# SJTU-ViSYS/TextSLAM

Measured on AMD Instinct MI355X. Metric: local_ba_residuals_per_s, higher is better.
Workload: dtype f64; 1 GPU; C4 local BA: 20 KF x 5000 pts x 100 text planes (541 (KF,plane) pairs x 64 features), passes 2,1,0 x <=10 LM its; parallelism=1 GPU, resid_evals_per_call=8113350

## Files before the change

### textslam_amd/csrc/tsba.hip

```cpp
#include <hip/hip_runtime.h>
#include <cstdio>
#include <cstdlib>
#include <cstring>
#include <cmath>
#include <string>
#include <vector>
#include <chrono>
#include <thread>
#include <mutex>
#include <map>
#include <condition_variable>
#include <atomic>
#include <functional>
#include <dlfcn.h>
#include <rccl/rccl.h>
#include "../../include/tsba.h"
#include "../../include/tsba_debug.h"
#include "tsba_device.h"
#include "tsraster.h"
#include "tsquadstat.h"
#include "tsba_plan.h"

#include "tsba_types.h"
#include "tsba_kernels_lin.h"
// ... 486 lines not shown
                set_err(c, "hipHostMalloc (plane cache staging)"); return TSBA_ERR_DEVICE; }
            IC.stage_cap = need; }
        for (size_t m = 0; m < miss.size(); m++) { const int k = miss[m];
            for (int l = 0; l < p->n_levels; l++) if (mask >> l & 1) memcpy(IC.stage + m*off + lo[l], p->img[l][k], (size_t)p->img_w[l]*p->img_h[l]);
            hipMemcpyAsync(IC.dev + (size_t)ic_slot[(size_t)k]*off, IC.stage + m*off, off, hipMemcpyHostToDevice, c->stream); }
    }
    c->use_img_cache = true;
    return 0;
}
static int stage_levels(Ctx *c, const tsba_problem *p, const tsba_options *o, const PlanStart &S, LevelMax *mx, UploadTimes &T) {
    if (S.first_plan) {
        flush_run(c);
        const auto tp0 = UpClock::now(); S.first_plan();
        T.plan += ms_between(tp0, UpClock::now()); }
    const std::vector<int> used = levels_used(o, p->n_levels);
    for (size_t i = 0; i < used.size(); i++) {
        const int l = used[i];
        if (S.defer && i > 0) { mx->take(level_capacity(p, l)); continue; }
        const int rc = stage_level(c, p, l, &T.plan, &T.img); if (rc) return rc;
        mx->take(level_size(c->lev[l]));
    }
    c->stage_p = S.defer ? p : nullptr;
    return 0;
}
static int alloc_pose_buffers(Ctx *c, const tsba_problem *p, const LevelMax &mx) {
    Work &W = c->W;
    c->pose_only = p->n_kf == 1 && every_landmark_frozen(p) && !c->dbg.no_pose_kernel;
    W.pst = nullptr; W.ppart = nullptr;
    if (c->pose_only) { AL(W.pst, 2); AL(W.ppart, 3*28*mx.pose_grid); }
    return 0;
}
static int alloc_lin_buffers(Ctx *c, const tsba_problem *p, const LevelMax &mx) {
    Work &W = c->W;
    for (int b = 0; b < 2; b++) {
        LinBuf &B = W.lb[b];
        AL(B.pairM, 27*mx.pair); AL(B.pairCost, mx.pair); AL(B.pairR, 9*mx.pair); AL(B.pairOut, 90*mx.pair);
        AL(B.tgM, 27*mx.tg); AL(B.tgCost, mx.tg);
        AL(B.w_pt, PT_REC*mx.pslot); AL(B.vdb_pt, PT_VDB*(size_t)p->n_pt);
        AL(B.w_tx, TX_REC*mx.tslot); AL(B.V_tx, 6*(size_t)p->n_text); AL(B.b_tx, 3*(size_t)p->n_text); AL(B.dgs_tx, 3*(size_t)p->n_text);
        AL(B.Hd, W.N); AL(B.bp, W.N); AL(B.bp_loc, W.N); AL(B.dgs_p, W.N);
        AL(B.lmpart, 3*((size_t)p->n_pt/64 + (size_t)p->n_text/2 + mx.pair + 8));
    }
    AL(W.sig_pt, p->n_pt); AL(W.sig_tx, 3*(size_t)p->n_text); AL(W.sig_p, W.N);
    AL(W.cb, 2*(size_t)W.N + 8); AL(W.cbm, 1);
    return 0;
}
static SolverLayout upload_layout(const Ctx *c) {
    int ring = 0, ring_k0 = 0; for (int l = 0; l < c->n_levels; l++) if (c->lev_built[l] && c->hplan[l].ring) { ring = 1; ring_k0 = c->hplan[l].ring_k0; }
    return choose_solver_layout(c->n_kf, max_band_rows(c), ring, ring_k0, is_multi(c), c->dbg);
}
static int alloc_reduced_system(Ctx *c, const tsba_problem *p, const SolverLayout &L) {
    Work &W = c->W; const int bw = L.bw_rows;
    c->lay = L;
    W.dp_poll = L.use_lds && !is_multi(c) && !c->pose_only && (c->dbg.solve_variant == 0 || c->dbg.solve_variant == 5 || c->dbg.solve_variant == 6);
    if (W.dp_poll) {
        const int ldsb = solve_back_lds_bytes((int)(solve_lds_doubles(W.N)*sizeof(double)), W.N);
        ATTR(k_solve_back<true>, ldsb);
        if (!grid_resident(c, (const void *)k_solve_back<true>, SOLVE_THREADS, (size_t)ldsb, 1 + (c->nb_back_max + 2)/3)) W.dp_poll = 0;
    }
    c->S_up = L.S_up; c->S_count = L.S_count; AL(c->S_alloc, c->S_count);
    if (!L.band) { W.S = c->S_alloc; W.ldS = W.N; W.band = 0; }
    else { W.S = c->S_alloc + (L.LDB - L.S_up); W.ldS = (int)L.LDB - 1; W.band = 1; }
    W.ring = 0; W.ring_g = 0; W.ring_b = 0; W.ring_k0 = -1;
    c->Lcol = nullptr; c->band_stream = L.band_stream; c->sep_cr = L.sep_cr != 0; c->band_parts = L.P;
    if (L.band_stream) AL(c->Lcol, ((size_t)p->n_kf + bw/6 + 1)*bw*6);
    if (L.partitioned) {
        const int P = L.P, nsep = L.nsep;
        c->nsep_ld = nsep;
        AL(c->Lb, ((size_t)p->n_kf + bw/6 + 1)*bw*6); AL(c->Tbuf, (size_t)P*((size_t)4*bw*bw + 2*bw));
        AL(c->Bpart, (size_t)P*BANDP_NS*((size_t)bw*bw + bw));
        if (L.sep_cr) { AL(c->Ssep, cr_pool_blocks(L.nsepb)*(size_t)bw*bw); AL(c->CRcontrib, (size_t)L.nsepb*cre_contrib_doubles(bw)); AL(c->CRfac, (size_t)L.nsepb*cre_rec_doubles(bw)); AL(c->CRgate, (size_t)(L.nsepb + 2)*TSBA_CRE_KMAX); c->cre_epoch = 0; }
        else AL(c->Ssep, (size_t)nsep*nsep + nsep);
        AL(c->Lcol_sep, (size_t)(nsep/6 + 1)*L.bws*6);
        Work &Ws = c->Wsep; memset(&Ws, 0, sizeof(Ws));
        Ws.N = nsep; Ws.n_kf = 0; Ws.S = c->Ssep; Ws.ldS = nsep; Ws.band = 1; Ws.st = nullptr;
        AL(Ws.Sy, nsep); AL(Ws.g, nsep); AL(Ws.dp, nsep); AL(Ws.LDbuf, 32*(size_t)(nsep/6 + 1)); AL(Ws.nfree, 1); AL(Ws.fidx, 1);
        W.ring = L.ring; W.ring_g = L.ring_G; W.ring_b = bw/6; W.ring_k0 = L.ring_k0;
    }
    if (L.err) { set_err(c, "ring-shaped map: the partitioned band solver is not available for this plan"); return L.err; }
    AL(W.Sy, W.N + BAND_BW_MAX);
    return 0;
}
static int alloc_pcg(Ctx *c, const tsba_problem *p, const SolverLayout &L) {
    Work &W = c->W;
    c->far_B = 0; c->n_far = 0; c->pcg_parts = 0;
    for (int l = 0; l < p->n_levels; l++) if (c->lev_built[l] && c->lev[l].far_B > 0) { c->far_B = c->lev[l].far_B; c->n_far = std::max(c->n_far, c->lev[l].n_far); }
    if (c->far_B > 0) {
        if (!W.band || !c->band_stream) { set_err(c, "map with long-range coupling: the band solvers are not available for this plan"); return TSBA_ERR_STATE; }
        c->pcg_parts = (p->n_kf + 31)/32;
        AL(W.Sfar, 36*(size_t)std::max(c->n_far, 1));
        AL(W.pc_x, W.N); AL(W.pc_r, W.N); AL(W.pc_p[0], W.N); AL(W.pc_p[1], W.N); AL(W.pc_q, W.N); AL(W.pc_g0, W.N);
        AL(W.pc_part, 5*(size_t)c->pcg_parts + 16 + 144); AL(W.pcs, 2); AL(W.pc_stat, 8);
    }
    c->S_xchg = nullptr; c->xchg_wp = L.xchg_wp;
    if (L.xchg_wp) AL(c->S_xchg, ((size_t)W.N + L.bw_rows)*L.xchg_wp);
    return 0;
}
static int alloc_step_buffers(Ctx *c, const tsba_problem *p, const LevelMax &mx) {
    Work &W = c->W;
    AL(W.g, W.N); AL(W.dp, W.N + 2); AL(W.dl_pt, p->n_pt); AL(W.dl_tx, 3*(size_t)p->n_text);
    AL(W.partial, 2*(size_t)c->nb_back_max);
    AL(W.posepart, 2*((size_t)p->n_kf/21 + 2));
    AL(W.cntpart, 2*(mx.cnt/4 + mx.cnt/256 + 4));
    AL(W.st, 2); c->st_base = W.st; AL(W.dec, 1);
    W.st_next = (W.dp_poll && p->n_kf <= SCHUR_KEEP_KF) ? W.st + 1 : nullptr;
    AL(c->cov_log, 6*TSBA_MAX_LEVELS);
    return 0;
// ... 242 lines not shown
        c->lin_base += grid;
        return;
    }
    if (D.n_pair + D.n_tg > 0) launch_k_linearize(c, D, spec);
    const MidDec md0{0, 0, 0, tsba_options{}};
    if (mid_threads(c) == MID_TW) LAUNCHK((k_mid<MID_TW, 6, MID_PR_MIN>), dim3(nb_pt + nb_tx + nb_pr), dim3(MID_TW), 0, c->stream, W, D, nb_pt, nb_tx, spec, md0);
    else if (mid_threads(c) == 64) {
        const int dec_on = spec && decision_in_mid(c, D) ? 1 : 0;
        LAUNCHK((k_mid<64, 6, MID_PR_MIN>), dim3(nb_pt + nb_tx + nb_pr + dec_on), dim3(64), 0, c->stream, W, D, nb_pt, nb_tx, spec,
                dec_on ? MidDec{1, nb_pr, back_blocks_pt(c->n_pt) + back_blocks_tx(c->n_text) + nb_kf, c->opt} : md0);
    } else LAUNCHK((k_mid<256, 4, MID_PR_MIN>), dim3(nb_pt + nb_tx + nb_pr), dim3(256), 0, c->stream, W, D, nb_pt, nb_tx, spec, md0);
    const int multi = is_multi(c);
    const int npp = pose_parts(c);
    if (multi) {
        if (npp) LAUNCHK(k_pose_sums_raw, dim3(npp), dim3(256), 0, c->stream, W, D, spec);
        LAUNCHK(k_sums_multi, dim3(1), dim3(256), 0, c->stream, W, D, spec, nb_pt + nb_tx + nb_pr, back_blocks_pt(c->n_pt) + back_blocks_tx(c->n_text) + nb_kf, back_blocks_pt(c->n_pt) + back_blocks_tx(c->n_text), npp);
        allreduce(c, W.cb, 2*(size_t)W.N + 8, ncclDouble, ncclSum);
        allreduce(c, W.cbm, 1, ncclDouble, ncclMax);
        if (npp) LAUNCHK(k_pose_scale_multi, dim3(npp), dim3(256), 0, c->stream, W, spec);
    } else if (npp) LAUNCHK(k_pose_sums, dim3(npp), dim3(256), 0, c->stream, W, D, spec);
    if (!spec && !skip_postlin) LAUNCHK(k_postlin, dim3(1), dim3(256), 0, c->stream, W, D, c->opt.gradient_tolerance, nb_pt + nb_tx + nb_pr, multi, npp);
}
static int solve_lds_bytes(Ctx *c, int *use_lds) {
    *use_lds = lds_solver_fits(c->W.N);
    return *use_lds ? (int)(solve_lds_doubles(c->W.N)*sizeof(double)) : 0;
}
static int chol_subst_lds_bytes() { return (CH_NB*(CH_NB + 1) + 2*CH_NB + 8*CH_NB)*(int)sizeof(double); }
static void launch_schur(Ctx *c, const LevelDev &D, int multi, SchurDec dec = SchurDec{0, 0, 0, tsba_options{}}) {
    if (c->n_kf > 126 && !c->dbg.no_schur_quad) {
        const int nq = D.n_sb > 0 ? (((D.n_sb + 3)/4 + 7)/8)*8 : 0, ng = ((c->n_kf + 7)/8)*8;
        if (D.n_tg > 0) LAUNCHK(k_schur_quad<true>, dim3(nq + ng), dim3(64), 0, c->stream, c->W, D, multi, nq, ng);
        else LAUNCHK(k_schur_quad<false>, dim3(nq + ng), dim3(64), 0, c->stream, c->W, D, multi, nq, ng);
    } else if (c->n_kf > 126) LAUNCHK(k_schur_t<1>, dim3(D.n_sb + c->n_kf), dim3(64), 0, c->stream, c->W, D, multi, 0, SchurDec{0, 0, 0, tsba_options{}});
    else LAUNCHK(k_schur_t<4>, dim3(D.n_sb + c->n_kf + (dec.on == 3 ? 1 : 0)), dim3(256), 0, c->stream, c->W, D, multi, 0, dec);
    if (D.far_B > 0 && D.n_far > 0) {
        LevelDev E = D;
        E.n_sb = D.n_far; E.sb_a = D.far_a; E.sb_b = D.far_b; E.sb_pab = D.fb_pab; E.sb_pba = D.fb_pba; E.sb_far = D.fb_id;
        E.sb_pt_off = D.fb_pt_off; E.sb_pt_s1 = D.fb_pt_s1; E.sb_pt_s2 = D.fb_pt_s2; E.sb_pt_lm = D.fb_pt_lm;
        E.sb_tx_off = D.fb_tx_off; E.sb_tx_s1 = D.fb_tx_s1; E.sb_tx_s2 = D.fb_tx_s2; E.sb_tx_lm = D.fb_tx_lm;
        if (c->n_kf > 126 && !c->dbg.no_schur_quad) { const int nq = (((E.n_sb + 3)/4 + 7)/8)*8;
            if (D.n_tg > 0) LAUNCHK(k_schur_quad<true>, dim3(nq), dim3(64), 0, c->stream, c->W, E, multi, nq, 0);
            else LAUNCHK(k_schur_quad<false>, dim3(nq), dim3(64), 0, c->stream, c->W, E, multi, nq, 0); }
        else if (c->n_kf > 126) LAUNCHK(k_schur_t<1>, dim3(E.n_sb), dim3(64), 0, c->stream, c->W, E, multi, 0, SchurDec{0, 0, 0, tsba_options{}});
        else LAUNCHK(k_schur_t<4>, dim3(E.n_sb), dim3(256), 0, c->stream, c->W, E, multi, 0, SchurDec{0, 0, 0, tsba_options{}});
    }
}
static int set_solver_attrs(Ctx *c) {
    int use_lds; int lds = solve_lds_bytes(c, &use_lds);
    if (use_lds) { ATTR(k_solve_t<false>, lds);
        ATTR((k_solve_t<false, false>), lds);
        ATTR(k_solve_back<true>, solve_back_lds_bytes(lds, c->W.N));
        ATTR(k_solve_back<false>, solve_back_lds_bytes(lds, c->W.N));
        ATTR((k_solve_back<true, true>), solve_back_lds_bytes(lds, c->W.N));
        ATTR(k_solve_la, (int)std::min<size_t>(solve_la_lds_doubles(c->W.N)*sizeof(double), 160*1024 - 64)); }
    else {
        ATTR(k_band_solve, 156*1024);
        ATTR(k_bandp_factor, 156*1024);
        ATTR(k_cr_pivot, 156*1024);
        ATTR(k_cr_update, 156*1024);
        ATTR(k_cr_back, 156*1024);
        ATTR(k_cre_elim, 156*1024);
        ATTR(k_bandp_sepf, 156*1024);
        ATTR(k_cre_back, 156*1024);
        ATTR(k_ms_cre_back, 159*1024);
        ATTR(k_ms_cre_fwd, 100*1024);
        ATTR(k_ms_cre_root, 100*1024);
        ATTR(k_sv_linv, 156*1024);
#define MX_ATTR(SS) ATTR(k_mx_cre_fwd<SS>, 156*1024); ATTR(k_mx_cre_root<SS>, 156*1024); ATTR(k_mx_cre_back<SS>, 156*1024);
        MX_ATTR(36) MX_ATTR(42) MX_ATTR(48) MX_ATTR(54) MX_ATTR(60) MX_ATTR(66)
#undef MX_ATTR
        ATTR(k_sv_fwd_int<1>, 156*1024); ATTR(k_sv_fwd_int<2>, 156*1024);
        ATTR(k_sv_back_int<1>, 156*1024); ATTR(k_sv_back_int<2>, 156*1024);
        ATTR(k_sv_tree_back<1>, 150*1024); ATTR(k_sv_tree_back<2>, 150*1024);
        ATTR(k_bandp_backsub<1>, 156*1024); ATTR(k_bandp_backsub<2>, 156*1024);
        ATTR(k_band_backsub<1>, 156*1024); ATTR(k_band_backsub<2>, 156*1024); ATTR(k_band_backsub<3>, 156*1024);
        ATTR(k_solve_t<true>, (int)(solve_diag_lds_doubles()*sizeof(double)));
        ATTR(k_chol_panel, (CH_NB + 64)*(CH_NB + 1)*(int)sizeof(double));
        ATTR(k_chol_update, 2*64*(CH_NB + 1)*(int)sizeof(double));
        ATTR(k_chol_backsub, chol_subst_lds_bytes()); ATTR(k_chol_fwd, chol_subst_lds_bytes());
    }
    return 0;
}
#include "tsba_solve_launch.h"

static bool fused_decisions(const Ctx *c, const LevelDev &D) { return c->W.st_next != nullptr && D.far_B <= 0; }
static bool window_fast_ctx(const Ctx *c, bool per_step) { return c->W.st_next != nullptr && c->n_kf <= 64 && !is_multi(c) && !c->pose_only && !per_step; }
static bool window_fast(const Ctx *c, const LevelDev &D, bool per_step) { return window_fast_ctx(c, per_step) && D.far_B <= 0 && D.n_sc + D.n_tg > 0; }
static void launch_decide(Ctx *c, const LevelDev &D) {
    Work &W = c->W;
    int nb_pt, nb_tx, nb_pr; mid_blocks(c, D, nb_pt, nb_tx, nb_pr); const int nb_kf = (c->n_kf + 255)/256;
    const int nb_all = back_blocks_pt(c->n_pt) + back_blocks_tx(c->n_text) + nb_kf;
    LAUNCHK(k_decide, dim3(1), dim3(256), 0, c->stream, W, D, nb_all, nb_pt + nb_tx + nb_pr, c->opt, (int)is_multi(c), pose_parts(c));
}
static void launch_step(Ctx *c, const LevelDev &D, bool decide_prev = false, bool first_fused = false) {
    struct XT { Ctx *c; size_t x0; ~XT() { c->x_trial = c->x_acc - x0; } } xt{c, c->x_acc};
    Work &W = c->W;
    int nb_pt, nb_tx, nb_pr; mid_blocks(c, D, nb_pt, nb_tx, nb_pr); const int nb_kf = (c->n_kf + 255)/256;
    if ((int64_t)D.n_sb < (int64_t)c->n_kf*(c->n_kf + 1)/2 && (!c->band_stream || c->S_stale || is_multi(c))) {
        hipMemsetAsync(c->S_alloc, 0, sizeof(double)*c->S_count, c->stream); c->S_stale = false;
        if (D.far_B > 0) hipMemsetAsync(W.Sfar, 0, sizeof(double)*36*(size_t)std::max(D.n_far, 1), c->stream); }
    const int bb_pt = back_blocks_pt(c->n_pt), bb_tx = back_blocks_tx(c->n_text), nb_all = bb_pt + bb_tx + nb_kf;
    const bool fused_decide = fused_decisions(c, D);
    if (fused_decide && (decide_prev || first_fused)) {
        launch_schur(c, D, 0, SchurDec{decide_prev ? (decision_in_mid(c, D) ? 3 : 1) : 2, nb_all, nb_pt + nb_tx + nb_pr, c->opt});
        std::swap(W.st, W.st_next);
    } else launch_schur(c, D, (int)is_multi(c));
    if (is_multi(c)) {
        if (c->S_xchg) {
            const size_t nx = ((size_t)W.N + (W.ring ? c->xchg_wp - 6 : 0))*c->xchg_wp;
            const int nbp = (int)std::min<size_t>(2048, (nx + 255)/256);
            LAUNCHK(k_band_pack, dim3(nbp), dim3(256), 0, c->stream, W, c->S_xchg, c->xchg_wp, 0);
            allreduce(c, c->S_xchg, nx, ncclDouble, ncclSum);
            LAUNCHK(k_band_pack, dim3(nbp), dim3(256), 0, c->stream, W, c->S_xchg, c->xchg_wp, 1);
        } else allreduce(c, c->S_alloc, c->S_count, ncclDouble, ncclSum);
        if (D.far_B > 0 && D.n_far > 0) allreduce(c, W.Sfar, 36*(size_t)D.n_far, ncclDouble, ncclSum);
        allreduce(c, W.g, W.N, ncclDouble, ncclSum);
        LAUNCHK(k_damp_multi, dim3((c->n_kf + 255)/256), dim3(256), 0, c->stream, W);
    }
    if (W.dp_poll && D.far_B <= 0) {
        int use_lds; const int lds = solve_lds_bytes(c, &use_lds);
        const int ldsb = solve_back_lds_bytes(lds, W.N);
        if (c->dbg.solve_variant == 6) LAUNCHK((k_solve_back<true, true>), dim3(1 + (nb_all + 2)/3), dim3(SOLVE_THREADS), ldsb, c->stream, W, D, bb_pt, bb_tx, nb_all);
        else if (c->dbg.solve_variant == 5) LAUNCHK(k_solve_back<false>, dim3(1 + (nb_all + 2)/3), dim3(SOLVE_THREADS), ldsb, c->stream, W, D, bb_pt, bb_tx, nb_all);
        else LAUNCHK(k_solve_back<true>, dim3(1 + (nb_all + 2)/3), dim3(SOLVE_THREADS), ldsb, c->stream, W, D, bb_pt, bb_tx, nb_all);
    } else {
        launch_solve_full(c, D);
        LAUNCHK(k_back, dim3(nb_all), dim3(256), 0, c->stream, W, D, bb_pt, bb_tx);
    }
    launch_linearize(c, D, 1);
    if (!fused_decide) launch_decide(c, D);
}

struct PassCarry {
    const bool per_step;
    bool log_pending = false;
    int ms_ahead = -1;
    bool clear_part = false;
};
static bool pose_path(const Ctx *c) { return c->pose_only && !is_multi(c); }
static bool converged(const Ctx *c, int it) {
    if (!c->hprog || is_multi(c)) return false;
    const auto tw = std::chrono::steady_clock::now();
    for (int spin = 0;; spin++) {
        const unsigned long long w = *(volatile unsigned long long *)c->hprog;
        if ((unsigned int)(w >> 32) == c->W.pass_seq) { if (w & 1) return true; if ((int)((w & 0xffffffffu) >> 1) + 2 > it) break; }
        else if (it < 2) break;
        PlanPool::cpu_relax();
        if ((spin & 1023) == 1023 && std::chrono::steady_clock::now() - tw > std::chrono::seconds(2)) break;
    }
    return false;
}
static int level_ready(Ctx *c, int l) {
    if (!c->lev_built[l]) {
        if (!c->stage_p) { set_err(c, "level not staged"); return TSBA_ERR_STATE; }
        c->stage_async = true; const int rc = stage_level(c, c->stage_p, l, nullptr, nullptr); c->stage_async = false; if (rc) return rc; }
    if (c->lev_wait[l]) { hipStreamWaitEvent(c->stream, c->ev_stage[l], 0); c->lev_wait[l] = 0; }
    return TSBA_OK;
}
static void record_cov(Ctx *c, int ps) { if (c->cov_text >= 0 && c->cov_text < c->n_text && ps < TSBA_MAX_LEVELS) LAUNCHK(k_record_vtx, dim3(1), dim3(64), 0, c->stream, c->W, c->cov_text, c->cov_log + 6*ps); }
static int pose_pass(Ctx *c, int ps, PassCarry &carry) {
    const tsba_options &o = c->opt; const LevelDev &D = c->lev[o.levels[ps]]; const int G = pose_grid(D);
    const bool one_launch = !carry.per_step && grid_resident(c, (const void *)k_pose_pass, POSE_WG, 0, G);
    c->W.hprog = c->hprog; c->W.pass_seq = ++c->pass_seq;
    LAUNCHK(k_pose_begin, dim3(D.n_tg + 1), dim3(MS_THREADS), 0, c->stream, c->W, D, o.initial_radius, o.its[ps], (const uint8_t *)c->kf_initial,
            one_launch ? c->W.ppart : (double *)nullptr, 3*28*G, carry.log_pending ? c->st_log + ps - 1 : (LmState *)nullptr);
    int k_last = -1;
    if (one_launch) LAUNCHK(k_pose_pass, dim3(G), dim3(POSE_WG), 0, c->stream, c->W, D, o, G, o.its[ps]);
    else {
        LAUNCHK(k_pose_iter, dim3(G), dim3(POSE_WG), 0, c->stream, c->W, D, o, -1, G);
        for (int k = 0; k <= o.its[ps]; k++) {
            if (k >= 1 && converged(c, k - 1)) break;
            LAUNCHK(k_pose_iter, dim3(G), dim3(POSE_WG), 0, c->stream, c->W, D, o, k, G); k_last = k;
        }
        if (k_last < 0) k_last = 0;
    }
// ... 594 lines not shown
```

### textslam_amd/csrc/tsba_kernels_step.h

```cpp
#pragma once
#define BK_TP 4
#define BK_TT 16
#define BK_PT (256/BK_TP)
#define BK_TX (256/BK_TT)
static inline int back_blocks_pt(int n_pt) { return (n_pt + BK_PT - 1)/BK_PT; }
static inline int back_blocks_tx(int n_text) { return (n_text + BK_TX - 1)/BK_TX; }
template <bool POLL>
__device__ __forceinline__ void back_body(const Work &W, const LevelDev &L, int nb_pt, int nb_tx, int b, int tid, bool live, double *red, double *dps) {
    LmState *st = W.st;
    const bool is_pt = live && b < nb_pt, is_tx = live && !is_pt && b < nb_pt + nb_tx;
    const int T = is_pt ? BK_TP : BK_TT, part = is_pt ? tid % BK_TP : tid % BK_TT;
    const int j = is_pt ? b*BK_PT + tid/BK_TP : is_tx ? (b - nb_pt)*BK_TX + tid/BK_TT : 0;
    const bool lm = (is_pt && j < W.n_pt) || (is_tx && j < W.n_text);
    int o = 0, e = 0, act_ = 0, a0[3] = {0, 0, 0};
    if (lm && is_pt) { o = L.pls_off[j]; e = L.pls_off[j+1]; act_ = W.act_pt[j];
#pragma unroll
        for (int u = 0; u < 3; u++) a0[u] = part + BK_TP*u < 6 ? L.pt_pose6[6*(size_t)j + part + BK_TP*u] : 0; }
    else if (lm) { o = L.tls_off[j]; e = L.tls_off[j+1]; act_ = W.act_tx[j]; }
    if (st->done) return;
    const int cur = st->cur;
    const double irad = 1.0/st->radius;
    bool fail = st->step_fail;
    const LinBuf &B = W.lb[st->lcur];
    const double *dp = W.dp;
// ... 115 lines not shown
                    for (int u = 0; u < TB; u++) if (slot_of(k0 + u) < e) tx_slot(a[u], w[u]);
                }
#pragma unroll
                for (int k = 0; k < 3; k++) { double t = acc[k];
#pragma unroll
                    for (int x = 1; x < BK_TT; x <<= 1) t += __shfl_xor(t, x, 64);
                    acc[k] = (POLL ? tq[k] : B.b_tx[(size_t)k*W.n_text + j]) + t; }
                double Vd[6], Vi[6], lam[3];
#pragma unroll
                for (int k = 0; k < 6; k++) Vd[k] = POLL ? tq[3 + k] : B.V_tx[(size_t)k*W.n_text + j];
#pragma unroll
                for (int k = 0; k < 3; k++) lam[k] = (POLL ? tq[9 + k] : B.dgs_tx[(size_t)k*W.n_text + j])*irad;
                Vd[0] += lam[0]; Vd[3] += lam[1]; Vd[5] += lam[2];
                if (inv_sym3(Vd, Vi)) {
                    d[0] = -(Vi[0]*acc[0] + Vi[1]*acc[1] + Vi[2]*acc[2]);
                    d[1] = -(Vi[1]*acc[0] + Vi[3]*acc[1] + Vi[4]*acc[2]);
                    d[2] = -(Vi[2]*acc[0] + Vi[4]*acc[1] + Vi[5]*acc[2]);
                    if (part == 0) for (int k = 0; k < 3; k++) { step2 += d[k]*d[k]; mcc += lam[k]*d[k]*d[k] - (POLL ? tq[k] : B.b_tx[(size_t)k*W.n_text + j])*d[k]; }
                }
            }
            if (part == 0) for (int k = 0; k < 3; k++) W.theta[cur ^ 1][3*j + k] = W.theta[cur][3*j + k] + d[k];
        }
    } else if (live) {
        int a = (b - nb_pt - nb_tx)*256 + tid;
        if (a < W.n_kf) {
            double xl[7];
#pragma unroll
            for (int k = 0; k < 7; k++) xl[k] = POLL ? tq[k] : W.pose[cur][7*a + k];
            const double *x = xl; double *c = W.pose[cur ^ 1] + 7*a;
            if (!fail && (POLL ? pfi : W.fidx[a]) >= 0) {
                double d[6];
#pragma unroll
                for (int k = 0; k < 6; k++) d[k] = dp[6*a + k];
                double q[4] = { x[0], x[1], x[2], x[3] }, qn[4];
                quat_plus(q, d, qn);
                for (int k = 0; k < 4; k++) { c[k] = qn[k]; step2 += (qn[k] - q[k])*(qn[k] - q[k]); }
                for (int k = 0; k < 3; k++) { c[4 + k] = x[4 + k] + d[3 + k]; step2 += d[3 + k]*d[3 + k]; }
                for (int k = 0; k < 6; k++) { const double lam = (POLL ? wq[0][k] : B.dgs_p[6*a + k])*irad; mcc += lam*d[k]*d[k] - (POLL ? wq[1][k] : B.bp[6*a + k])*d[k]; }
            } else for (int k = 0; k < 7; k++) c[k] = x[k];
        }
    }
    red[tid] = step2; red[256 + tid] = mcc; __syncthreads();
    if (tid < 64) {
        double sv = ((red[tid] + red[tid + 64]) + red[tid + 128]) + red[tid + 192], sm = ((red[256 + tid] + red[256 + tid + 64]) + red[256 + tid + 128]) + red[256 + tid + 192];
        sv = wave_sum1(sv); sm = wave_sum1(sm);
        if (tid == 0 && live) { W.partial[2*b] = sv; W.partial[2*b + 1] = sm; }
    }
}
__global__ __launch_bounds__(256) void k_back(Work W, LevelDev L, int nb_pt, int nb_tx) {
    __shared__ double red[512];
    back_body<false>(W, L, nb_pt, nb_tx, blockIdx.x, threadIdx.x, true, red, nullptr);
}
#define BACK_RED 512
template <bool RL = true, bool OLD = false>
__global__ __launch_bounds__(SOLVE_THREADS) void k_solve_back(Work W, LevelDev L, int nb_pt, int nb_tx, int nb_all) {
    extern __shared__ __attribute__((aligned(16))) double smem[];
    if (blockIdx.x != 0) {
        const int sub = threadIdx.x >> 8, b = 3*((int)blockIdx.x - 1) + sub;
        back_body<true>(W, L, nb_pt, nb_tx, b, threadIdx.x & 255, b < nb_all, smem + BACK_RED*sub, smem + 3*BACK_RED);
        return; }
    solve_body<false, true, RL, OLD>(W, 0, smem);
}
static inline int solve_back_lds_bytes(int solver_bytes, int N) { return std::max(solver_bytes, (int)((3*BACK_RED + N + 2)*sizeof(double))); }

template <class S>
__device__ __forceinline__ double lm_decide(S &s, double cost, double step2, double mcc, double gmax_c, double xn_c, const tsba_options &o) {
    double verdict = 0.0;
    mcc *= 0.5;
    s.it++;
    s.cand_cost = cost; s.model_change = mcc; s.step_norm = sqrt(step2);
    if (s.step_fail || !(mcc > 0.0)) {
        s.step_fail = 0; verdict = -1.0;
        if (++s.invalid >= 5) { s.done = 1; s.term = 5; return verdict; }
        s.radius *= 0.5;
    } else {
        s.invalid = 0; s.n_cost++;
        if (!(cost == cost)) cost = 1.7976931348623157e308;
        if (s.step_norm <= o.parameter_tolerance*(s.x_norm + o.parameter_tolerance)) { s.done = 1; s.term = 2; return 2.0; }
        double cost_change = s.x_cost - cost;
        if (fabs(cost_change) <= o.function_tolerance*s.x_cost) { s.done = 1; s.term = 1; return 2.0; }
        double rel = cost_change/mcc;
        if (rel > o.min_relative_decrease) {
            s.cur ^= 1; s.lcur ^= 1; s.accepted++; s.n_lin++;
            s.x_cost = cost; s.x_norm = sqrt(xn_c); s.gmax = gmax_c;
            double t = 2.0*rel - 1.0, f = 1.0 - t*t*t; if (f < 1.0/3.0) f = 1.0/3.0;
            s.radius = fmin(s.radius/f, o.max_radius);
            s.decrease_factor = 2.0; verdict = 1.0;
            if (gmax_c <= o.gradient_tolerance) { s.done = 1; s.term = 3; return verdict; }
        } else {
            s.radius = s.radius/s.decrease_factor; s.decrease_factor *= 2.0;
        }
    }
    if (s.it >= s.max_it) { s.done = 1; s.term = 0; }
    else if (s.radius < o.min_radius) { s.done = 1; s.term = 4; }
    return verdict;
}
__device__ __forceinline__ void lm_decide_publish(const Work &W, const LmState &s, double cost, double mcc_half, double verdict) {
    if (W.trace && s.it >= 1 && s.it <= TSBA_TRACE_CAP) {
        double *t = W.trace + 4*((size_t)W.trace_pass*TSBA_TRACE_CAP + s.it - 1);
        t[0] = verdict < 0.0 ? __longlong_as_double(0x7ff8000000000000LL) : (cost == cost ? cost : 1.7976931348623157e308); t[1] = mcc_half; t[2] = s.radius; t[3] = verdict; }
    if (W.hprog) { *W.hprog = ((unsigned long long)W.pass_seq << 32) | ((unsigned long long)s.it << 1) | (s.done ? 1u : 0u); __threadfence_system(); }
}
__device__ __forceinline__ void decide_body(const Work &W, const LevelDev &L, int nb_back, int nb_lm, const tsba_options &o, int multi, int npp) {
    LmState *st = W.st;
    if (W.dp_poll) for (int k = threadIdx.x; k <= W.N; k += 256) W.dp[k] = __builtin_nan("");
    if (st->done) return;
    __shared__ double red[5*256], xch[256];
    const int tid = threadIdx.x;
    const LinBuf &Bc = W.lb[st->lcur ^ 1];
    double gmax_c, xn_c, cost;
    double step2 = 0.0, mcc = 0.0;
#ifdef TSBA_SOLVE_STAMPS
    const long long s0_ = clock64(); long long s1_ = 0, s2_ = 0, s3_ = 0;
#endif
// ... 223 lines not shown
```

### textslam_amd/csrc/tsba_solve.h

```cpp
#pragma once

#define SOLVE_THREADS 768
#define SOLVE_PW 2
#define SOLVE_PROWS (64 - 6)
#ifdef TSBA_SOLVE_STAMPS
__device__ long long ts_step_stamps[4*32];
#define STAMP(v) do { long long t_ = clock64(); v += t_ - tx; tx = t_; } while (0)
#else
#define STAMP(v) do { } while (0)
#endif
#define SOLVE_LD 48
#define LD_D 16
#define LD_ID 22
#define LD_M 28
typedef double v4d __attribute__((ext_vector_type(4)));
typedef double v2d __attribute__((ext_vector_type(2)));

__host__ __device__ __forceinline__ int tri(int i) { return (i*(i + 1)) >> 1; }
__host__ __device__ __forceinline__ int rowoff(int i) { return ((i + 1) >> 1)*((i >> 1) + 1)*2; }
__device__ __forceinline__ int tri_row(int e) {
    int i = (int)((__fsqrt_rn(8.f*(float)e + 1.f) - 1.f)*0.5f);
    if (tri(i) > e) i--; else if (tri(i + 1) <= e) i++;
    return i;
}
__device__ __forceinline__ double rcp_nr(double d) {
    double x = __builtin_amdgcn_rcp(d);
    double e = fma(-d, x, 1.0); x = fma(x, e, x);
    e = fma(-d, x, 1.0); x = fma(x, e, x);
    return x;
}
__device__ __forceinline__ double readlane_f64(double v, int src) {
    int lo = __builtin_amdgcn_readlane(__double2loint(v), src), hi = __builtin_amdgcn_readlane(__double2hiint(v), src);
    return __hiloint2double(hi, lo);
}
__device__ __forceinline__ void wave_lds_fence() {
    __builtin_amdgcn_fence(__ATOMIC_RELEASE, "wavefront");
    __builtin_amdgcn_wave_barrier();
    __builtin_amdgcn_fence(__ATOMIC_ACQUIRE, "wavefront");
}
__device__ __forceinline__ void ld6(const double *p, double v[6]) {
    const v2d a = ((const v2d *)p)[0], b = ((const v2d *)p)[1], c = ((const v2d *)p)[2];
    v[0] = a.x; v[1] = a.y; v[2] = b.x; v[3] = b.y; v[4] = c.x; v[5] = c.y;
}
__device__ __forceinline__ void st6(double *p, const double v[6]) {
    ((v2d *)p)[0] = v2d{v[0], v[1]}; ((v2d *)p)[1] = v2d{v[2], v[3]}; ((v2d *)p)[2] = v2d{v[4], v[5]};
}
__device__ __forceinline__ void ldl6(double s[21], double l[15], double d[6], double id[6], bool &bad) {
#pragma unroll
    for (int c = 0; c < 6; c++) {
        double dc = s[tri(c) + c];
        if (!(dc > 0.0)) { bad = true; dc = 1.0; }
        d[c] = dc; id[c] = rcp_nr(dc);
#pragma unroll
        for (int r = c + 1; r < 6; r++) {
            const double v = s[tri(r) + c], lr = v*id[c];
            l[tri(r - 1) + c] = lr;
#pragma unroll
            for (int q = c + 1; q <= r; q++) s[tri(r) + q] = fma(-lr, s[tri(q) + c], s[tri(r) + q]);
        }
    }
}
__device__ __forceinline__ void ldl6_lanes(const double a[6], double l[15], double d[6], double id[6], bool &bad) {
    double sd[6];
#pragma unroll
    for (int c = 0; c < 6; c++) sd[c] = a[c];
#pragma unroll
    for (int c = 0; c < 6; c++) {
        double dc = readlane_f64(sd[c], c);
        if (!(dc > 0.0)) { bad = true; dc = 1.0; }
        d[c] = dc; id[c] = rcp_nr(dc);
        double col[6];
#pragma unroll
// ... 40 lines not shown
                for (int k = 0; k < 8; k++) { const v2d x = ((const v2d *)o)[k]; t[2*k] = x.x; t[2*k + 1] = x.y; }
#pragma unroll
                for (int k = 0; k < 15; k++) m[k] = t[k];
            };
            auto step = [&](int q, const double col[w + 1][6], const double m[15]) {
                double zb[6], x[6];
#pragma unroll
                for (int c = 0; c < 6; c++) zb[c] = readlane_f64(z[w], 6*q + c);
#pragma unroll
                for (int c = 0; c < 6; c++) {
                    double v0 = zb[c], v1 = 0.0;
#pragma unroll
                    for (int k = c + 1; k < 6; k++) { if ((k - c) & 1) v0 = fma(m[tri(k - 1) + c], zb[k], v0); else v1 = fma(m[tri(k - 1) + c], zb[k], v1); }
                    x[c] = v0 + v1;
                }
                if (lane == 0) st6(rhs + 6*(10*w + q), x);
#pragma unroll
                for (int u = 0; u <= w; u++)
                    z[u] -= fma(col[u][0], x[0], fma(col[u][1], x[1], col[u][2]*x[2])) + fma(col[u][3], x[3], fma(col[u][4], x[4], col[u][5]*x[5]));
            };
            int q = min(9, nfree - 1 - 10*w);
            if constexpr (w < 2) {
                double colA[w + 1][6], mA[15], colB[w + 1][6], mB[15];
                fetch(q, colA, mA);
                for (; q >= 1; q -= 2) {
                    fetch(q - 1, colB, mB);
                    step(q, colA, mA);
                    if (q >= 2) fetch(q - 2, colA, mA);
                    step(q - 1, colB, mB);
                }
                if (q == 0) step(0, colA, mA);
            } else {
                double col[w + 1][6], m[15];
                for (; q >= 0; q--) { fetch(q, col, m); step(q, col, m); }
            }
        };
        if (nfree > 30) back(IC<3>{});
        if (nfree > 20) back(IC<2>{});
        if (nfree > 10) back(IC<1>{});
        back(IC<0>{});
}
__device__ __forceinline__ void solve_backsub_wave(double *A, double *LD, int n, int nfree, int lane) {
    solve_backsub_wave_ro(A, LD, n, nfree, lane, [](int i) { return rowoff(i); });
}

#define SOLVE_DIAG_NB 96
static size_t solve_lds_doubles(int N) { return (size_t)rowoff(N + 1) + 16 + (size_t)SOLVE_LD*(N/6) + 36*SOLVE_PW + 8; }
static bool lds_solver_fits(int N) { return solve_lds_doubles(N)*sizeof(double) <= 160*1024 - 64; }
static size_t solve_diag_lds_doubles() { return solve_lds_doubles(SOLVE_DIAG_NB) + rowoff(SOLVE_DIAG_NB + 1) + SOLVE_DIAG_NB + 36*(SOLVE_DIAG_NB/6) + 16; }


__device__ __forceinline__ double co_load(const double *p) { return __hip_atomic_load(p, __ATOMIC_RELAXED, __HIP_MEMORY_SCOPE_AGENT); }
__device__ __forceinline__ void co_store(double *p, double v) { __hip_atomic_store(p, v == v ? v : __builtin_inf(), __ATOMIC_RELAXED, __HIP_MEMORY_SCOPE_AGENT); }
template <bool DIAG, bool PUB, bool RL = true, bool OLD = false>
__device__ __forceinline__ void solve_body(const Work &W, int B0, double *smem) {
    LmState *st = W.st;
    __shared__ int fail;
    const int tid = threadIdx.x, lane = tid & 63, wave = __builtin_amdgcn_readfirstlane(tid >> 6);
    constexpr int NW = SOLVE_THREADS/64, NT = NW - SOLVE_PW;
    constexpr bool ROWS = !DIAG && !OLD;
#ifdef TSBA_SOLVE_STAMPS
    const long long Tl = clock64();
#endif
    const int Nmax = W.N;
    double *A = smem;
    const size_t ldS = (size_t)W.ldS;
    const double *Sb = DIAG ? W.S + (size_t)B0*ldS + B0 : W.S;
    const int rmax = DIAG ? Nmax - 1 - B0 : Nmax - 1;
    int done, nfree_all, sfail, nfree, n;
    double *LD, *scr;
    if constexpr (ROWS) {
        constexpr int P0 = 10, P1 = 4;
        constexpr int C0 = 6, LW0 = SOLVE_PW, LNW = NW - LW0;
        const bool loader = wave >= LW0;
        const int wl = wave - LW0;
        const int i0p = lane < 6 ? lane : 6 + wave*SOLVE_PROWS + lane - 6;
        const int gk = C0 + tid - 64*LW0;
        double v0[P0], v1[P1], gv = 0.0, pv[6], pg[6];
        if (loader) {
#pragma unroll
            for (int u = 0; u < P0; u++) { const int r = min(C0 + wl + LNW*u, rmax); v0[u] = Sb[(size_t)r*ldS + min(C0 + lane, r)]; }
#pragma unroll
            for (int u = 0; u < P1; u++) { const int r = min(C0 + 64 + wl + LNW*u, rmax); v1[u] = Sb[(size_t)r*ldS + min(C0 + 64 + lane, r)]; }
            gv = W.g[min(gk, Nmax - 1)];
        } else {
#pragma unroll
            for (int c = 0; c < 6; c++) { const int r = min(i0p, rmax); pv[c] = Sb[(size_t)r*ldS + min(c, r)]; pg[c] = W.g[min(c, Nmax - 1)]; }
        }
        done = st->done; nfree_all = *W.nfree; sfail = st->step_fail;
        if (done) return;
        nfree = nfree_all; n = 6*nfree;
        LD = A + rowoff(n + 1) + 16; scr = LD + SOLVE_LD*nfree;
        if (loader) {
#pragma unroll
            for (int u = 0; u < P0; u++) { const int r = C0 + wl + LNW*u, c = C0 + lane; if (r < n && c <= r) A[rowoff(r) + c] = v0[u]; }
#pragma unroll
            for (int u = 0; u < P1; u++) { const int r = C0 + 64 + wl + LNW*u, c = C0 + 64 + lane; if (r < n && c <= r) A[rowoff(r) + c] = v1[u]; }
            for (int ch = 0; C0 + 64*ch < n; ch++) {
                const int c = C0 + 64*ch + lane;
                for (int r0 = C0 + 64*ch + wl + LNW*(ch == 0 ? P0 : ch == 1 ? P1 : 0); r0 < n; r0 += 4*LNW) {
                    double w[4];
#pragma unroll
                    for (int u = 0; u < 4; u++) { const int r = min(r0 + LNW*u, n - 1); w[u] = Sb[(size_t)r*ldS + min(c, r)]; }
#pragma unroll
                    for (int u = 0; u < 4; u++) { const int r = r0 + LNW*u; if (r < n && c <= r) A[rowoff(r) + c] = w[u]; }
                }
            }
            if (gk < n) A[rowoff(n) + gk] = gv;
        } else {
            if (i0p < n) {
                if (lane >= 6) st6(A + rowoff(i0p), pv);
                else {
#pragma unroll
                    for (int c = 0; c < 6; c++) if (c <= lane) A[rowoff(i0p) + c] = pv[c];
                }
            } else if (i0p == n) st6(A + rowoff(n), pg);
            if (lane >= 6)
                for (int i = i0p + SOLVE_PW*SOLVE_PROWS; i <= n; i += SOLVE_PW*SOLVE_PROWS) {
#pragma unroll
                    for (int c = 0; c < 6; c++) pv[c] = i < n ? Sb[(size_t)i*ldS + c] : W.g[c];
                    st6(A + rowoff(i), pv);
                }
            wave_lds_fence();
        }
        if (tid == 0) fail = sfail;
    } else {
    const int neMax = DIAG ? tri(SOLVE_DIAG_NB) : tri(Nmax);
    double v[12]; int er[12], ec[12];
#pragma unroll
    for (int u = 0; u < 12; u++) {
        const int e = min(u*SOLVE_THREADS + tid, neMax - 1);
        er[u] = tri_row(e); ec[u] = e - tri(er[u]);
        v[u] = Sb[(size_t)min(er[u], rmax)*ldS + min(ec[u], rmax)];
    }
    done = st->done; nfree_all = *W.nfree; sfail = st->step_fail;
    if (done) return;
    if (DIAG && (sfail || 6*nfree_all <= B0)) return;
    nfree = DIAG ? min(SOLVE_DIAG_NB, 6*nfree_all - B0)/6 : nfree_all;
    n = 6*nfree;
    const int ne = tri(n);
    LD = A + rowoff(n + 1) + 16;
    scr = LD + SOLVE_LD*nfree;
#pragma unroll
    for (int u = 0; u < 12; u++) if (u*SOLVE_THREADS + tid < ne) A[rowoff(er[u]) + ec[u]] = v[u];
    for (int base = 12*SOLVE_THREADS; base < ne; base += 12*SOLVE_THREADS) {
#pragma unroll
        for (int u = 0; u < 12; u++) {
            const int e = min(base + u*SOLVE_THREADS + tid, ne - 1);
            er[u] = tri_row(e); ec[u] = e - tri(er[u]);
            v[u] = Sb[(size_t)er[u]*ldS + ec[u]];
        }
#pragma unroll
        for (int u = 0; u < 12; u++) if (base + u*SOLVE_THREADS + tid < ne) A[rowoff(er[u]) + ec[u]] = v[u];
    }
    for (int k = tid; k < n; k += SOLVE_THREADS) A[rowoff(n) + k] = DIAG ? 0.0 : W.g[k];
    if (tid == 0) fail = DIAG ? 0 : sfail;
    __syncthreads();
    }
#ifdef TSBA_SOLVE_STAMPS
    if (tid == 0) W.dbg[0] = clock64() - Tl;
    if (tid == 64*SOLVE_PW) W.dbg[3] = clock64() - Tl;
    long long tx = clock64(), T0 = tx, ta = 0, tb = 0, tc = 0, td = 0;
#endif
    for (int jb = 0; jb < nfree && !(jb == 0 ? (DIAG ? 0 : sfail) : fail); jb++) {
        const int j0 = 6*jb, R0 = j0 + 6, p0 = j0 - 6;
#ifdef TSBA_SOLVE_STAMPS
        const long long tx0_ = clock64();
#endif
        if (wave < SOLVE_PW) {
            double Lk[36], dprev[6];
            if (jb > 0) {
                ld6(LD + SOLVE_LD*(jb - 1) + LD_D, dprev);
#pragma unroll
                for (int c = 0; c < 6; c++) ld6(A + rowoff(j0 + c) + p0, Lk + 6*c);
            }
            auto load_row = [&](int i, double a[6]) {
                const double *row = A + rowoff(i);
                ld6(row + j0, a);
                if (jb > 0) {
                    double y[6];
                    ld6(row + p0, y);
#pragma unroll
                    for (int k = 0; k < 6; k++) y[k] *= dprev[k];
#pragma unroll
                    for (int c = 0; c < 6; c++) {
                        double v0 = y[0]*Lk[c*6], v1 = y[1]*Lk[c*6 + 1];
                        v0 = fma(y[2], Lk[c*6 + 2], v0); v1 = fma(y[3], Lk[c*6 + 3], v1);
                        v0 = fma(y[4], Lk[c*6 + 4], v0); v1 = fma(y[5], Lk[c*6 + 5], v1);
                        a[c] -= v0 + v1;
                    }
                }
            };
            const int i0 = lane < 6 ? j0 + lane : R0 + wave*SOLVE_PROWS + lane - 6;
            double a[6];
            load_row(min(i0, n), a);
            double l[15], d[6], id[6]; bool bad = false;
#ifdef TSBA_SOLVE_STAMPS
            long long sa_ = 0;
#endif
            if constexpr (RL) {
                STAMP(ta);
#ifdef TSBA_SOLVE_STAMPS
                sa_ = clock64();
#endif
                ldl6_lanes(a, l, d, id, bad);
            } else {
            if (lane < 6) st6(scr + wave*36 + lane*6, a);
            wave_lds_fence();
            STAMP(ta);
#ifdef TSBA_SOLVE_STAMPS
            sa_ = clock64();
#endif
            double s[21];
            {
                double t[36];
#pragma unroll
                for (int r = 0; r < 6; r++) ld6(scr + wave*36 + r*6, t + 6*r);
#pragma unroll
                for (int r = 0; r < 6; r++)
#pragma unroll
                    for (int c = 0; c <= r; c++) s[tri(r) + c] = t[6*r + c];
            }
            ldl6(s, l, d, id, bad);
            }
            if (wave == 0 && lane == 0) {
                double *o = LD + SOLVE_LD*jb;
#pragma unroll
                for (int k = 0; k < 15; k++) o[k] = l[k];
                st6(o + LD_D, d); st6(o + LD_ID, id);
                if (bad) { fail = 1; st->step_fail = 1; }
            }
            STAMP(tb);
#ifdef TSBA_SOLVE_STAMPS
            const long long sb_ = clock64();
#endif
            auto solve_row = [&](int i, double a[6]) {
#pragma unroll
                for (int c = 0; c < 5; c++)
#pragma unroll
                    for (int q = c + 1; q < 6; q++) a[q] = fma(-a[c], l[tri(q - 1) + c], a[q]);
#pragma unroll
                for (int c = 0; c < 6; c++) a[c] *= id[c];
                st6(A + rowoff(i) + j0, a);
            };
            if (lane >= 6) {
                if (i0 <= n) solve_row(i0, a);
                for (int i = i0 + SOLVE_PW*SOLVE_PROWS; i <= n; i += SOLVE_PW*SOLVE_PROWS) { load_row(i, a); solve_row(i, a); }
            }
#ifdef TSBA_SOLVE_STAMPS
            if (!DIAG && wave == 0 && lane == 0 && jb < 32) { const long long se_ = clock64(); ts_step_stamps[jb] = sa_ - tx0_; ts_step_stamps[32 + jb] = sb_ - sa_; ts_step_stamps[64 + jb] = se_ - sb_; }
#endif
            if (wave == 1 && jb == nfree - 1) {
                double m[15];
                inv_unit_lower6(l, m);
                if (lane == 0) {
#pragma unroll
                    for (int k = 0; k < 15; k++) LD[SOLVE_LD*jb + LD_M + k] = m[k];
                }
            }
        } else if (jb > 0) {
            const int mr = n - R0 + 1, mc = n - R0;
            const double *ldp = LD + SOLVE_LD*(jb - 1);
            if (mc > 0) {
                const int ntr = (mr + 15) >> 4, ntc = (mc + 15) >> 4, ntile = tri(ntr);
                const int lr = lane & 15, lk = lane >> 4;
                const int k1 = min(4 + lk, 5);
                const double dk0 = ldp[LD_D + lk], dk1 = lk < 2 ? ldp[LD_D + 4 + lk] : 0.0;
                for (int t = wave - SOLVE_PW; t < ntile; t += NT) {
                    const int ti = tri_row(t), tj = t - tri(ti);
                    if (tj >= ntc) continue;
                    const int arow = rowoff(min(R0 + 16*ti + lr, n)) + p0, brow = rowoff(min(R0 + 16*tj + lr, n - 1)) + p0;
                    double a0 = -A[arow + lk], a1 = -A[arow + k1];
                    double b0 = A[brow + lk]*dk0, b1 = A[brow + k1]*dk1;
                    if (lk >= 2) { a1 = 0.0; b1 = 0.0; }
                    const int ccol = R0 + 16*tj + lr;
                    v4d c; int ci[4]; bool ok[4];
#pragma unroll
                    for (int r = 0; r < 4; r++) {
                        const int crow = R0 + 16*ti + lk + 4*r;
                        ok[r] = crow <= n && ccol <= crow && ccol < n;
                        ci[r] = rowoff(min(crow, n)) + min(ccol, min(crow, n - 1));
                        c[r] = A[ci[r]];
                    }
                    c = __builtin_amdgcn_mfma_f64_16x16x4f64(a0, b0, c, 0, 0, 0);
                    c = __builtin_amdgcn_mfma_f64_16x16x4f64(a1, b1, c, 0, 0, 0);
#pragma unroll
                    for (int r = 0; r < 4; r++) if (ok[r]) A[ci[r]] = c[r];
                }
            }
            if (wave == NW - 1) {
                double l[15], m[15];
#pragma unroll
                for (int k = 0; k < 15; k++) l[k] = ldp[k];
                inv_unit_lower6(l, m);
                if (lane == 0) {
#pragma unroll
                    for (int k = 0; k < 15; k++) LD[SOLVE_LD*(jb - 1) + LD_M + k] = m[k];
                }
            }
        }
        STAMP(tc);
#ifdef TSBA_SOLVE_STAMPS
        if (!DIAG && lane == 0 && jb < 32) { const long long se_ = clock64();
            if (wave == 2) ts_step_stamps[3*32 + jb] = se_ - tx0_; }
#endif
        __syncthreads();
        STAMP(td);
    }
#ifdef TSBA_SOLVE_STAMPS
    if (lane == 0 && (wave == 0 || wave == 2 || wave == NW - 1)) {
        long long *o = W.dbg + 8 + 4*(wave == 0 ? 0 : wave == 2 ? 1 : 2); o[0] = ta; o[1] = tb; o[2] = tc; o[3] = td;
        if (wave == 0) { W.dbg[1] = clock64() - T0; W.dbg[6] = nfree; }
    }
    long long T1 = clock64();
#endif
    if (DIAG) {
        if (fail) return;
        double *Mi = scr + 36*SOLVE_PW;
        double *sq = Mi + rowoff(SOLVE_DIAG_NB + 1), *tmp = sq + SOLVE_DIAG_NB;
        for (int t = tid; t < 21*nfree; t += SOLVE_THREADS) {
            const int b = t/21, e = t - 21*b, r = tri_row(e), q = e - tri(r);
            Mi[rowoff(6*b + r) + 6*b + q] = r == q ? 1.0 : LD[SOLVE_LD*b + LD_M + tri(r - 1) + q];
        }
        for (int t = tid; t < n; t += SOLVE_THREADS) sq[t] = sqrt(LD[SOLVE_LD*(t/6) + LD_D + t % 6]);
        __syncthreads();
        for (int b = 1; b < nfree; b++) {
            const int nout = 36*b;
            for (int t = tid; t < nout; t += SOLVE_THREADS) {
                const int c = t/36, r = (t - 36*c)/6, q = t % 6;
                double acc = 0.0;
                const double *lrow = A + rowoff(6*b + r);
                for (int k = 6*c + q; k < 6*b; k++) acc = fma(lrow[k], Mi[rowoff(k) + 6*c + q], acc);
                tmp[t] = acc;
            }
            __syncthreads();
            for (int t = tid; t < nout; t += SOLVE_THREADS) {
                const int c = t/36, r = (t - 36*c)/6, q = t % 6;
                double acc = tmp[36*c + 6*r + q];
                for (int m = 0; m < r; m++) acc = fma(LD[SOLVE_LD*b + LD_M + tri(r - 1) + m], tmp[36*c + 6*m + q], acc);
                Mi[rowoff(6*b + r) + 6*c + q] = -acc;
// ... 51 lines not shown
```

Before: 1.809 billion residuals/s.

## Precompute per-wave tile plan and batch MFMA trailing updates in LDS Cholesky

The trailing-update phase of the in-LDS dense factorization now uses a per-wave tile assignment, precomputed at compile time and bit-packed in constant memory. This replaces the per-tile sqrt-based tri_row decode. Row offsets come from cheap incremental arithmetic with a fast path for full interior tiles, and tiles are processed in batches of up to three so all loads are issued before the MFMAs, which raises instruction-level parallelism. The per-step fail check is dropped from the loop condition, and the plan caps each wave at eight tiles, so larger systems or mid-factorization failures may behave differently. The old path stays available as solve variant 7.

```diff
diff --git a/textslam_amd/csrc/tsba.hip b/textslam_amd/csrc/tsba.hip
--- a/textslam_amd/csrc/tsba.hip
+++ b/textslam_amd/csrc/tsba.hip
@@ -562,7 +562,7 @@
 static int alloc_reduced_system(Ctx *c, const tsba_problem *p, const SolverLayout &L) {
     Work &W = c->W; const int bw = L.bw_rows;
     c->lay = L;
-    W.dp_poll = L.use_lds && !is_multi(c) && !c->pose_only && (c->dbg.solve_variant == 0 || c->dbg.solve_variant == 5 || c->dbg.solve_variant == 6);
+    W.dp_poll = L.use_lds && !is_multi(c) && !c->pose_only && (c->dbg.solve_variant == 0 || c->dbg.solve_variant == 5 || c->dbg.solve_variant == 6 || c->dbg.solve_variant == 7);
     if (W.dp_poll) {
         const int ldsb = solve_back_lds_bytes((int)(solve_lds_doubles(W.N)*sizeof(double)), W.N);
         ATTR(k_solve_back<true>, ldsb);
@@ -911,6 +911,7 @@
         ATTR(k_solve_back<true>, solve_back_lds_bytes(lds, c->W.N));
         ATTR(k_solve_back<false>, solve_back_lds_bytes(lds, c->W.N));
         ATTR((k_solve_back<true, true>), solve_back_lds_bytes(lds, c->W.N));
+        ATTR((k_solve_back<true, false, true>), solve_back_lds_bytes(lds, c->W.N));
         ATTR(k_solve_la, (int)std::min<size_t>(solve_la_lds_doubles(c->W.N)*sizeof(double), 160*1024 - 64)); }
     else {
         ATTR(k_band_solve, 156*1024);
@@ -980,6 +981,7 @@
         int use_lds; const int lds = solve_lds_bytes(c, &use_lds);
         const int ldsb = solve_back_lds_bytes(lds, W.N);
         if (c->dbg.solve_variant == 6) LAUNCHK((k_solve_back<true, true>), dim3(1 + (nb_all + 2)/3), dim3(SOLVE_THREADS), ldsb, c->stream, W, D, bb_pt, bb_tx, nb_all);
+        else if (c->dbg.solve_variant == 7) LAUNCHK((k_solve_back<true, false, true>), dim3(1 + (nb_all + 2)/3), dim3(SOLVE_THREADS), ldsb, c->stream, W, D, bb_pt, bb_tx, nb_all);
         else if (c->dbg.solve_variant == 5) LAUNCHK(k_solve_back<false>, dim3(1 + (nb_all + 2)/3), dim3(SOLVE_THREADS), ldsb, c->stream, W, D, bb_pt, bb_tx, nb_all);
         else LAUNCHK(k_solve_back<true>, dim3(1 + (nb_all + 2)/3), dim3(SOLVE_THREADS), ldsb, c->stream, W, D, bb_pt, bb_tx, nb_all);
     } else {
diff --git a/textslam_amd/csrc/tsba_kernels_step.h b/textslam_amd/csrc/tsba_kernels_step.h
--- a/textslam_amd/csrc/tsba_kernels_step.h
+++ b/textslam_amd/csrc/tsba_kernels_step.h
@@ -191,14 +191,14 @@
     back_body<false>(W, L, nb_pt, nb_tx, blockIdx.x, threadIdx.x, true, red, nullptr);
 }
 #define BACK_RED 512
-template <bool RL = true, bool OLD = false>
+template <bool RL = true, bool OLD = false, bool TOLD = false>
 __global__ __launch_bounds__(SOLVE_THREADS) void k_solve_back(Work W, LevelDev L, int nb_pt, int nb_tx, int nb_all) {
     extern __shared__ __attribute__((aligned(16))) double smem[];
     if (blockIdx.x != 0) {
         const int sub = threadIdx.x >> 8, b = 3*((int)blockIdx.x - 1) + sub;
         back_body<true>(W, L, nb_pt, nb_tx, b, threadIdx.x & 255, b < nb_all, smem + BACK_RED*sub, smem + 3*BACK_RED);
         return; }
-    solve_body<false, true, RL, OLD>(W, 0, smem);
+    solve_body<false, true, RL, OLD, TOLD>(W, 0, smem);
 }
 static inline int solve_back_lds_bytes(int solver_bytes, int N) { return std::max(solver_bytes, (int)((3*BACK_RED + N + 2)*sizeof(double))); }
 
diff --git a/textslam_amd/csrc/tsba_solve.h b/textslam_amd/csrc/tsba_solve.h
--- a/textslam_amd/csrc/tsba_solve.h
+++ b/textslam_amd/csrc/tsba_solve.h
@@ -16,8 +16,7 @@
 typedef double v4d __attribute__((ext_vector_type(4)));
 typedef double v2d __attribute__((ext_vector_type(2)));
 
-__host__ __device__ __forceinline__ int tri(int i) { return (i*(i + 1)) >> 1; }
-__host__ __device__ __forceinline__ int rowoff(int i) { return ((i + 1) >> 1)*((i >> 1) + 1)*2; }
+#include "tsba_solve_tiles.h"
 __device__ __forceinline__ int tri_row(int e) {
     int i = (int)((__fsqrt_rn(8.f*(float)e + 1.f) - 1.f)*0.5f);
     if (tri(i) > e) i--; else if (tri(i + 1) <= e) i++;
@@ -164,12 +163,16 @@
 
 __device__ __forceinline__ double co_load(const double *p) { return __hip_atomic_load(p, __ATOMIC_RELAXED, __HIP_MEMORY_SCOPE_AGENT); }
 __device__ __forceinline__ void co_store(double *p, double v) { __hip_atomic_store(p, v == v ? v : __builtin_inf(), __ATOMIC_RELAXED, __HIP_MEMORY_SCOPE_AGENT); }
-template <bool DIAG, bool PUB, bool RL = true, bool OLD = false>
+__constant__ const unsigned long long solve_tile_plans[SOLVE_TILE_WAVES] = {solve_tile_plan(0), solve_tile_plan(1), solve_tile_plan(2), solve_tile_plan(3),
+    solve_tile_plan(4), solve_tile_plan(5), solve_tile_plan(6), solve_tile_plan(7), solve_tile_plan(8), solve_tile_plan(9)};
+template <bool DIAG, bool PUB, bool RL = true, bool OLD = false, bool TOLD = false>
 __device__ __forceinline__ void solve_body(const Work &W, int B0, double *smem) {
     LmState *st = W.st;
     __shared__ int fail;
     const int tid = threadIdx.x, lane = tid & 63, wave = __builtin_amdgcn_readfirstlane(tid >> 6);
     constexpr int NW = SOLVE_THREADS/64, NT = NW - SOLVE_PW;
+    static_assert(NT == SOLVE_TILE_WAVES, "the tile plan is laid out for ten update waves");
+    const unsigned long long plan = solve_tile_plans[wave >= SOLVE_PW ? wave - SOLVE_PW : 0];
     constexpr bool ROWS = !DIAG && !OLD;
 #ifdef TSBA_SOLVE_STAMPS
     const long long Tl = clock64();
@@ -274,7 +277,12 @@
     if (tid == 64*SOLVE_PW) W.dbg[3] = clock64() - Tl;
     long long tx = clock64(), T0 = tx, ta = 0, tb = 0, tc = 0, td = 0;
 #endif
-    for (int jb = 0; jb < nfree && !(jb == 0 ? (DIAG ? 0 : sfail) : fail); jb++) {
+    const int nsteps = !DIAG && sfail ? 0 : nfree;
+    const int lr = lane & 15, lk = lane >> 4;
+    const SolveLaneRow xr = solve_lane_row(lr), xk = solve_lane_row(lk);
+    const int ron = rowoff(n), ron1 = rowoff(n - 1);
+    int tcnt = SOLVE_TILE_KMAX;
+    for (int jb = 0; jb < nsteps && (!TOLD || !(jb > 0 && fail)); jb++) {
         const int j0 = 6*jb, R0 = j0 + 6, p0 = j0 - 6;
 #ifdef TSBA_SOLVE_STAMPS
         const long long tx0_ = clock64();
@@ -375,9 +383,67 @@
             const double *ldp = LD + SOLVE_LD*(jb - 1);
             if (mc > 0) {
                 const int ntr = (mr + 15) >> 4, ntc = (mc + 15) >> 4, ntile = tri(ntr);
-                const int lr = lane & 15, lk = lane >> 4;
+                const double dk0 = ldp[LD_D + lk], dk1 = lk < 2 ? ldp[LD_D + 4 + lk] : 0.0;
+                if constexpr (!TOLD) {
+                tcnt = solve_tile_count(plan, tcnt, ntr);
+                const int live = solve_tile_live(plan, tcnt, ntc);
+                const double *Ap = A + p0 + lk;
+                auto batch = [&](auto NBC, int k0) {
+                    constexpr int NB = decltype(NBC)::value;
+                    double a0[NB], a1[NB], b0[NB], b1[NB]; v4d c[NB]; int ci[NB][4]; bool full[NB], ok[NB][4];
+#pragma unroll
+                    for (int u = 0; u < NB; u++) {
+                        const int e = solve_tile_entry(plan, k0 + u), ti = e & 15, tj = e >> 4;
+                        const int ba = R0 + 16*ti, bb = R0 + 16*tj;
+                        const int ha = solve_tile_half_sq(ba), hb = solve_tile_half_sq(bb);
+                        const int ccol = bb + lr;
+                        int arow, brow;
+                        full[u] = tj < ti && ba + 15 <= n;
+                        if (full[u]) {
+                            arow = solve_tile_rowoff_in(ba, ha, xr); brow = solve_tile_rowoff_in(bb, hb, xr);
+                            solve_tile_rowoff4_in(ba, ha, xk, ci[u]);
+#pragma unroll
+                            for (int r = 0; r < 4; r++) { ci[u][r] += ccol; ok[u][r] = true; }
+                        } else {
+                            arow = solve_tile_rowoff(ba, ha, xr, n, ron); brow = solve_tile_rowoff(bb, hb, xr, n - 1, ron1);
+                            bool past[4];
+                            solve_tile_rowoff4(ba, ha, xk, n, ron, ci[u], past);
+#pragma unroll
+                            for (int r = 0; r < 4; r++) {
+                                const int cmax = min(ba + lk + 4*r, n - 1);
+                                ok[u][r] = !past[r] && ccol <= cmax;
+                                ci[u][r] += min(ccol, cmax);
+                            }
+                        }
+                        a0[u] = Ap[arow]; a1[u] = Ap[arow + 4];
+                        b0[u] = Ap[brow]; b1[u] = Ap[brow + 4];
+#pragma unroll
+                        for (int r = 0; r < 4; r++) c[u][r] = A[ci[u][r]];
+                    }
+                    __builtin_amdgcn_sched_barrier(0);
+#pragma unroll
+                    for (int u = 0; u < NB; u++) {
+                        a0[u] = -a0[u]; a1[u] = -a1[u]; b0[u] *= dk0; b1[u] *= dk1;
+                        if (lk >= 2) { a1[u] = 0.0; b1[u] = 0.0; }
+                        c[u] = __builtin_amdgcn_mfma_f64_16x16x4f64(a0[u], b0[u], c[u], 0, 0, 0);
+                        c[u] = __builtin_amdgcn_mfma_f64_16x16x4f64(a1[u], b1[u], c[u], 0, 0, 0);
+                    }
+#pragma unroll
+                    for (int u = 0; u < NB; u++) {
+                        if (full[u]) {
+#pragma unroll
+                            for (int r = 0; r < 4; r++) A[ci[u][r]] = c[u][r];
+                        } else {
+#pragma unroll
+                            for (int r = 0; r < 4; r++) if (ok[u][r]) A[ci[u][r]] = c[u][r];
+                        }
+                    }
+                };
+                int k0 = 0;
+                for (; k0 + 3 <= live; k0 += 3) batch(IC<3>{}, k0);
+                if (live - k0 == 2) batch(IC<2>{}, k0); else if (live - k0 == 1) batch(IC<1>{}, k0);
+                } else {
                 const int k1 = min(4 + lk, 5);
-                const double dk0 = ldp[LD_D + lk], dk1 = lk < 2 ? ldp[LD_D + 4 + lk] : 0.0;
                 for (int t = wave - SOLVE_PW; t < ntile; t += NT) {
                     const int ti = tri_row(t), tj = t - tri(ti);
                     if (tj >= ntc) continue;
@@ -398,6 +464,7 @@
                     c = __builtin_amdgcn_mfma_f64_16x16x4f64(a1, b1, c, 0, 0, 0);
 #pragma unroll
                     for (int r = 0; r < 4; r++) if (ok[r]) A[ci[r]] = c[r];
+                }
                 }
             }
             if (wave == NW - 1) {
diff --git a/textslam_amd/csrc/tsba_solve_tiles.h b/textslam_amd/csrc/tsba_solve_tiles.h
--- /dev/null
+++ b/textslam_amd/csrc/tsba_solve_tiles.h
@@ -0,0 +1,62 @@
+#pragma once
+#if defined(__HIPCC__)
+#define TS_HD __host__ __device__ __forceinline__
+#else
+#define TS_HD inline
+#endif
+
+TS_HD constexpr int tri(int i) { return (i*(i + 1)) >> 1; }
+TS_HD constexpr int rowoff(int i) { return ((i + 1) >> 1)*((i >> 1) + 1)*2; }
+
+#define SOLVE_TILE_WAVES 10
+#define SOLVE_TILE_KMAX 8
+TS_HD constexpr unsigned long long solve_tile_plan(int wl) {
+    unsigned long long p = 0;
+    int t = 0, ti = 0, tj = 0;
+    for (int k = 0; k < SOLVE_TILE_KMAX; k++) {
+        for (; t < wl + SOLVE_TILE_WAVES*k; t++) if (++tj > ti) { ti++; tj = 0; }
+        p |= (unsigned long long)(ti | tj << 4) << 8*k;
+    }
+    return p;
+}
+TS_HD constexpr int solve_tile_entry(unsigned long long plan, int k) { return (int)(plan >> 8*k) & 255; }
+TS_HD constexpr int solve_tile_ti(unsigned long long plan, int k) { return solve_tile_entry(plan, k) & 15; }
+TS_HD constexpr int solve_tile_tj(unsigned long long plan, int k) { return solve_tile_entry(plan, k) >> 4; }
+TS_HD constexpr int solve_tile_count(unsigned long long plan, int cnt, int ntr) {
+    while (cnt > 0 && solve_tile_ti(plan, cnt - 1) >= ntr) cnt--;
+    return cnt;
+}
+TS_HD constexpr int solve_tile_live(unsigned long long plan, int cnt, int ntc) { return cnt - (cnt > 0 && solve_tile_tj(plan, cnt - 1) >= ntc ? 1 : 0); }
+
+TS_HD int solve_mul24(int a, int b) {
+#if defined(__HIP_DEVICE_COMPILE__)
+    return (int)__umul24((unsigned)a, (unsigned)b);
+#else
+    return a*b;
+#endif
+}
+struct SolveLaneRow { int x1, rox; };
+TS_HD SolveLaneRow solve_lane_row(int x) { return SolveLaneRow{x + 1, rowoff(x)}; }
+TS_HD int solve_tile_half_sq(int b) { return (b*b) >> 1; }
+TS_HD int solve_tile_rowoff_in(int b, int hsq, SolveLaneRow x) { return hsq + solve_mul24(b, x.x1) + x.rox; }
+TS_HD int solve_tile_rowoff(int b, int hsq, SolveLaneRow x, int nclamp, int ron) {
+    const int o = hsq + solve_mul24(b, x.x1) + x.rox;
+    return b + x.x1 - 1 <= nclamp ? o : ron;
+}
+TS_HD void solve_tile_rowoff4_in(int b, int hsq, SolveLaneRow x, int out[4]) {
+    const int i0 = b + x.x1 - 1;
+    int o = hsq + solve_mul24(b, x.x1) + x.rox, d = 4*i0 + 12;
+    out[0] = o;
+#ifdef __HIPCC__
+#pragma unroll
+#endif
+    for (int r = 1; r < 4; r++) { o += d; d += 16; out[r] = o; }
+}
+TS_HD void solve_tile_rowoff4(int b, int hsq, SolveLaneRow x, int nclamp, int ron, int out[4], bool past[4]) {
+    const int i0 = b + x.x1 - 1;
+    int o = hsq + solve_mul24(b, x.x1) + x.rox, d = 4*i0 + 12;
+#ifdef __HIPCC__
+#pragma unroll
+#endif
+    for (int r = 0; r < 4; r++) { past[r] = i0 + 4*r > nclamp; out[r] = past[r] ? ron : o; o += d; d += 16; }
+}
```

After: 1.821 billion residuals/s (median of 5 runs). About the same (+0.6%).
